# Arieys/MonteCarloPathTracing

Hardware: AMD Instinct MI355X
Metric: Mrays/s on cornell-box 1280x720 SPP=256 (closest-hit queries actually traced / wall time incl. gather) (higher is better)
Workload: dtype f64

## Files before the change

montecarlopathtracing_amd/csrc/kernels.hip:

```cpp
#include <hip/hip_runtime.h>

#include "accel_build.hpp"
#include "dev_common.hpp"
#include "kernels.hpp"
#include "shade_common.hpp"
#include "shade_path.hpp"
#include "trace_persistent.hpp"
#include "trace_pool.hpp"

namespace mcpt {

template <bool LEAF>
__global__ void __launch_bounds__(256) k_trace_closest_reference(DScene S, const double* __restrict__ rays, long long n,
                                                       int32_t* __restrict__ face, double* __restrict__ t_out,
                                                       double* __restrict__ p_out, double* __restrict__ pn_out, DCounters* ctr)
{
    const long long gid = (long long)blockIdx.x * blockDim.x + threadIdx.x;
    LaneStats ls;
    if (gid < n) {
        Ray r;
        r.o = ld3(rays + gid * 6); r.d = ld3(rays + gid * 6 + 3);
        Hit h; Work w = {0, 0};
        const bool ok = trace_closest(S, r, h, w);
        ls.nodes = w.nodes; ls.tris = w.tris; ls.primary = 1;
        V3 pn = mk(0, 0, 0);
        if (ok && !LEAF) pn = hit_normal(S, h);
        if (face) face[gid] = ok ? (LEAF ? h.leaf : S.tris[h.leaf].face) : -1;
        if (t_out) t_out[gid] = ok ? h.t : 0.0;
        if (p_out) { p_out[gid * 3] = h.p.x; p_out[gid * 3 + 1] = h.p.y; p_out[gid * 3 + 2] = h.p.z; }
        if (pn_out) { pn_out[gid * 3] = pn.x; pn_out[gid * 3 + 1] = pn.y; pn_out[gid * 3 + 2] = pn.z; }
    }
    flush_stats(ctr, ls);
}

struct ArrayRaySource {
    static constexpr bool kWantsPoint = true;
    const double* rays; long long n;
    int32_t* leaf_out; double* t_out; double* p_out;
    __device__ __forceinline__ long long total() const { return n; }
    __device__ __forceinline__ bool fetch(long long q, Ray& r) const
    {
        r.o = ld3(rays + q * 6); r.d = ld3(rays + q * 6 + 3);
#ifdef MCPT_DBG_INVALID
        return ((((unsigned int)q * 2654435761u) >> 7) & 3u) != 0u;
#else
        return true;
#endif
    }
    __device__ __forceinline__ void store(long long q, bool ok, const Hit& h) const
    {
        leaf_out[q] = ok ? h.leaf : -1;
        t_out[q] = ok ? h.t : 0.0;
        p_out[q * 3] = h.p.x; p_out[q * 3 + 1] = h.p.y; p_out[q * 3 + 2] = h.p.z;
    }
};

struct PrimaryRaySource {
    static constexpr bool kWantsPoint = true;
    const double* dirs; const int32_t* pixels; int n_pixels; double eye[3]; PrimaryHit* hits;
    __device__ __forceinline__ long long total() const { return n_pixels; }
    __device__ __forceinline__ bool fetch(long long q, Ray& r) const
    {
        const int pix = pixels ? pixels[q] : (int)q;
        r.o = ld3(eye); r.d = ld3(dirs + (size_t)pix * 3);
        return true;
    }
    __device__ __forceinline__ void store(long long q, bool ok, const Hit& h) const
    {
        PrimaryHit ph;
        ph.leaf = ok ? h.leaf : -1; ph.surf = 0; ph.t = h.t; ph.p[0] = h.p.x; ph.p[1] = h.p.y; ph.p[2] = h.p.z;
        hits[q] = ph;
    }
};

template <class Src, int STACK, int WAVES>
__global__ void __launch_bounds__(256, WAVES) k_trace_persistent(DScene S, Src src, TraceQueue* queue, long long* slow_list, unsigned int slow_cap,
                                                                long long chunk, DCounters* ctr)
{
    __shared__ int lds_stack[STACK * 256];
    __shared__ double lds_rays[4 * MCPT_RAYBUF_BYTES / 8];
    LaneStats ls;
    Work w = {0, 0};
    trace_persistent(S, src, queue, slow_list, slow_cap, chunk, lds_stack + threadIdx.x, 256, lds_rays + (threadIdx.x >> 6) * (MCPT_RAYBUF_BYTES / 8), w, S.fast.stack_cap < STACK ? S.fast.stack_cap : STACK);
    ls.nodes = w.nodes; ls.tris = w.tris;
    { const unsigned long long tw = wave_sum(w.pre_wrong); if ((threadIdx.x & 63) == 0 && tw && ctr) atomicAdd(&ctr->pre_wrong, tw); }
    flush_stats(ctr, ls);
}

template <class Src, int NW, int KT, int SCAP>
__global__ void __launch_bounds__(NW * 64, 1) k_trace_pool(DScene S, Src src, TraceQueue* queue, long long* slow_list, unsigned int slow_cap,
                                                          long long chunk, DCounters* ctr)
{
    __shared__ PoolLds<NW, KT, SCAP> L;
    LaneStats ls;
    Work w = {0, 0};
    trace_pool<Src, NW, KT, SCAP>(S, src, queue, slow_list, slow_cap, chunk, L, w, reinterpret_cast<int*>(slow_list + slow_cap));
    ls.nodes = w.nodes; ls.tris = w.tris;
    { const unsigned long long tw = wave_sum(w.pre_wrong); if ((threadIdx.x & 63) == 0 && tw && ctr) atomicAdd(&ctr->pre_wrong, tw); }
    flush_stats(ctr, ls);
}

template <class Src>
__global__ void __launch_bounds__(256) k_trace_slow(DScene S, Src src, const TraceQueue* queue, const long long* slow_list, unsigned int slow_cap,
                                                    DCounters* ctr)
{
    __shared__ int lds_stack[MCPT_FAST_STACK * 256];
    LaneStats ls;
    Work w = {0, 0};
    trace_slow_list(S, src, queue, slow_list, slow_cap, w, lds_stack + threadIdx.x);
    ls.nodes = w.nodes; ls.tris = w.tris;
    flush_stats(ctr, ls);
}

__global__ void k_finish_hits(DScene S, long long n, int32_t* __restrict__ face, const double* __restrict__ p, double* __restrict__ pn_out, DCounters* ctr)
{
    const long long gid = (long long)blockIdx.x * blockDim.x + threadIdx.x;
    LaneStats ls;
    if (gid < n) {
        ls.primary = 1;
        const int leaf = face[gid];
        V3 pn = mk(0, 0, 0);
        if (leaf >= 0) {
            Hit h; h.leaf = leaf; h.t = 0; h.p = ld3(p + gid * 3);
            pn = hit_normal(S, h);
            face[gid] = S.tris[leaf].face;
        }
        if (pn_out) { pn_out[gid * 3] = pn.x; pn_out[gid * 3 + 1] = pn.y; pn_out[gid * 3 + 2] = pn.z; }
    }
    flush_stats(ctr, ls);
}

__global__ void k_primary_dirs(DCamera cam, double* __restrict__ dirs)
{
    const int row = blockIdx.x * blockDim.x + threadIdx.x;
    if (row >= cam.height) return;
    const V3 eye = ld3(cam.eye), pdx = ld3(cam.pdx);
    V3 pos = ld3(cam.start_point) - ld3(cam.pdy) * (double)row;
    double* out = dirs + (size_t)row * cam.width * 3;
    for (int j = 0; j < cam.width; j++) {
        const V3 d = normalized(pos - eye);
        out[j * 3] = d.x; out[j * 3 + 1] = d.y; out[j * 3 + 2] = d.z;
// ... 484 lines not shown
```

montecarlopathtracing_amd/csrc/trace_pool.hpp:

```cpp
#pragma once
#include "env.hpp"
#include "trace_persistent.hpp"
#include "vertex.hpp"

namespace mcpt {

struct NoPaths { static constexpr bool kPaths = false; };

#ifndef MCPT_POOL_WAVES
#define MCPT_POOL_WAVES 16
#endif
#ifndef MCPT_POOL_KT
#define MCPT_POOL_KT 20
#endif
#ifndef MCPT_POOL_STACK
#define MCPT_POOL_STACK 8
#endif
#define MCPT_POOL_SPILL (MCPT_FAST_STACK - MCPT_POOL_STACK)
#ifndef MCPT_POOL_CLAIMS
#define MCPT_POOL_CLAIMS 2
#endif
#define MCPT_POOL_CLAIM_ORDER __ATOMIC_ACQUIRE
#define MCPT_POOL_FILE_ORDER __ATOMIC_RELEASE

struct alignas(16) PoolOxy { double ox, oy; };
struct alignas(16) PoolOzDx { double oz, dx; };
struct alignas(16) PoolDyz { double dy, dz; };
struct alignas(16) PoolRcp { float rx, ry, rz, limit; };
typedef double pool_d2 __attribute__((ext_vector_type(2)));
template <class T>
__device__ __forceinline__ T pool_ld16(const T* p)
{
    static_assert(sizeof(T) == 16, "16-byte group");
    const pool_d2 v = *reinterpret_cast<const pool_d2*>(p);
    T r;
    __builtin_memcpy(&r, &v, 16);
    return r;
}

template <int NW, int KT, int SCAP>
struct PoolLds {
    PoolOxy oxy[KT * 64];
    PoolOzDx ozdx[KT * 64];
    PoolDyz dyz[KT * 64];
    PoolRcp rcp[KT * 64];
    double best_t[KT * 64];
    unsigned int q[KT * 64];
    int cur[KT * 64];
    int best_leaf[KT * 64];
    int spf[KT * 64];
    int stack[SCAP * KT * 64];
    unsigned int cls[5 * 64];
    unsigned int busy[64];
    int tbl[NW * 64];
    unsigned int stat[8];
    unsigned int live;
    unsigned int dry;
};

__device__ __forceinline__ int uni(int v) { return __builtin_amdgcn_readfirstlane(v); }
__device__ __forceinline__ long long uni(long long v)
{
    const int lo = __builtin_amdgcn_readfirstlane((int)(unsigned int)(unsigned long long)v);
    const int hi = __builtin_amdgcn_readfirstlane((int)(unsigned int)((unsigned long long)v >> 32));
    return (long long)(((unsigned long long)(unsigned int)hi << 32) | (unsigned int)lo);
}

template <class Src, int NW, int KT, int SCAP, class PP = NoPaths>
__device__ __forceinline__ void trace_pool(const DScene& S, const Src& src, TraceQueue* queue, long long* __restrict__ slow_list,
                                           unsigned int slow_cap, long long chunk, PoolLds<NW, KT, SCAP>& L, Work& w,
                                           int* __restrict__ spill ,
                                           const PP& pp = PP())
{
    static_assert(KT <= 32, "one 32-bit set per class");
    static_assert(SCAP >= 6, "the pushes of a ray's first two steps land in LDS");
    enum { C_INNER = 0, C_LEAF = 1, C_EXACT = 2, C_FIN = 3, C_SHADE = 4, C_DEAD = 5 };
    enum { F_FOUND = 256, F_AMBIG = 512, F_RAY = 1024, F_OWNFAIL = 2048  };
    const DFast& F = S.fast;
    const CwNode* __restrict__ nodes = F.cw;
    const DTri* __restrict__ tris = F.tris;
    const DTriPre* __restrict__ pre = F.pre;
    const TicketSchedule ts = make_ticket_schedule(src.total(), chunk);
    const int lane = threadIdx.x & 63, wave = uni((int)(threadIdx.x >> 6));
    const int stack_max = spill ? SCAP + MCPT_POOL_SPILL : SCAP;
    const int stack_cap = F.stack_cap < stack_max ? F.stack_cap : stack_max;
    int* __restrict__ my_spill = spill ? spill + (size_t)blockIdx.x * MCPT_POOL_SPILL * (KT * 64) : nullptr;
    auto st_put = [&](int e, int k, int v) __attribute__((always_inline)) {
        if (e < SCAP) L.stack[(e * KT + k) * 64 + lane] = v;
        else my_spill[((e - SCAP) * KT + k) * 64 + lane] = v;
    };
    auto st_get = [&](int e, int k) __attribute__((always_inline)) -> int {
        return e < SCAP ? L.stack[(e * KT + k) * 64 + lane] : my_spill[((e - SCAP) * KT + k) * 64 + lane];
    };

    for (int k = wave; k < KT; k += NW) { L.spf[k * 64 + lane] = 0; if constexpr (PP::kPaths) L.q[k * 64 + lane] = 0u; }
    int R = 1, NP = KT;
    if constexpr (PP::kPaths) { R = pp.nl + 1; NP = KT / R; }
    if (wave == 0) {
        L.cls[C_INNER * 64 + lane] = 0u; L.cls[C_LEAF * 64 + lane] = 0u; L.cls[C_EXACT * 64 + lane] = 0u;
        L.cls[C_FIN * 64 + lane] = PP::kPaths ? 0u : (unsigned int)((1ull << KT) - 1ull);
        L.cls[C_SHADE * 64 + lane] = PP::kPaths ? (unsigned int)((1ull << NP) - 1ull) : 0u;
        L.busy[lane] = 0u;
    }
    if (threadIdx.x == 0) { L.live = (PP::kPaths ? NP : KT) * 64; L.dry = 0; }
    if (threadIdx.x < 8) L.stat[threadIdx.x] = 0u;
    __syncthreads();

    unsigned int c_nodes = 0, c_rays = 0, c_exact = 0;
#ifdef MCPT_POOL_DEBUG
    unsigned long long d_used = 0, d_okc = 0, d_steps = 0, d_kill = 0, d_tickets = 0;
    unsigned long long d_cs[5] = {0, 0, 0, 0, 0}, d_cl[5] = {0, 0, 0, 0, 0}, d_sleep = 0, d_miss = 0, d_want[5] = {0, 0, 0, 0, 0};
    unsigned long long d_cyc[6] = {0, 0, 0, 0, 0, 0};
    unsigned long long d_t = __builtin_amdgcn_s_memtime();
    const unsigned long long d_t0 = d_t;
#endif
    long long next = 0, range_end = 0;
    bool queue_empty = false;
    int rot = wave % KT;
    const int rot_stride = (int)((0x13110d0bu >> (8 * ((wave >> 1) & 3))) & 255u) % KT | 1;
    const float s3f = __double2float_ru(3.0 * F.absmax), absmax_f = __double2float_ru(F.absmax);
    auto pad_of = [&](float of, float rf_) __attribute__((always_inline)) { return (0x1p-20f * 1.00001f) * ((fabsf(of) + s3f) * fabsf(rf_)); };
    auto margin_of = [&](const float of[3], const PoolRcp& a4) __attribute__((always_inline)) {
        const float rmax = fmaxf(fmaxf(fabsf(a4.rx), fabsf(a4.ry)), fabsf(a4.rz));
        const float scale = fmaxf(fmaxf(absmax_f, fabsf(of[0])), fmaxf(fabsf(of[1]), fabsf(of[2])));
        return rmax <= 0.99e6f ? (1.0000001e-9f * 1.00001f) * (scale * rmax) : __builtin_inff();
    };
    auto pop_next = [&](int idx, int k, int spf) __attribute__((always_inline)) -> int {
        int sp = spf & 255;
        if (sp == 0) return C_FIN;
        sp--;
        int nxt;
        if (!__ballot(sp >= SCAP)) { nxt = L.stack[(sp * KT + k) * 64 + lane]; __asm__ volatile("" : "+v"(nxt)); }
        else nxt = st_get(sp, k);
        const bool node = nxt >= 0;
        const int ref = -1 - nxt;
        const int first = node ? nxt : ref >> 4, cnt = (ref & 7) + 1;
        L.cur[idx] = first;
        L.spf[idx] = (spf & 0xff00) | sp | (node ? 0 : cnt << 16);
        return node ? C_INNER : C_LEAF;
    };

    for (;;) {
        const unsigned int m_inner = __hip_atomic_load(&L.cls[C_INNER * 64 + lane], __ATOMIC_RELAXED, __HIP_MEMORY_SCOPE_WORKGROUP);
        const unsigned int m_leaf = __hip_atomic_load(&L.cls[C_LEAF * 64 + lane], __ATOMIC_RELAXED, __HIP_MEMORY_SCOPE_WORKGROUP);
        const unsigned int m_exact = __hip_atomic_load(&L.cls[C_EXACT * 64 + lane], __ATOMIC_RELAXED, __HIP_MEMORY_SCOPE_WORKGROUP);
        const unsigned int m_fin = __hip_atomic_load(&L.cls[C_FIN * 64 + lane], __ATOMIC_RELAXED, __HIP_MEMORY_SCOPE_WORKGROUP);
        const int n_inner = __popcll(__ballot(m_inner != 0u));
        const int n_leaf = __popcll(__ballot(m_leaf != 0u));
        const int n_exact = __popcll(__ballot(m_exact != 0u));
        const bool fin_ok = PP::kPaths || !queue_empty || uni((int)__hip_atomic_load(&L.dry, __ATOMIC_RELAXED, __HIP_MEMORY_SCOPE_WORKGROUP)) == NW;
        const int n_fin = fin_ok ? __popcll(__ballot(m_fin != 0u)) : 0;
        unsigned int m_shade = 0u;
        int n_shade = 0;
        if constexpr (PP::kPaths) {
            m_shade = __hip_atomic_load(&L.cls[C_SHADE * 64 + lane], __ATOMIC_RELAXED, __HIP_MEMORY_SCOPE_WORKGROUP);
            n_shade = __popcll(__ballot(m_shade != 0u));
        }
        if (!(n_inner | n_leaf | n_exact | n_fin | n_shade)) {
            if (uni((int)__hip_atomic_load(&L.live, __ATOMIC_RELAXED, __HIP_MEMORY_SCOPE_WORKGROUP)) == 0) break;
            __builtin_amdgcn_s_sleep(4);
#ifdef MCPT_POOL_DEBUG
            d_sleep++;
#endif
            continue;
        }
        int c = C_FIN, best_score = n_fin;
        if (n_exact > best_score) { c = C_EXACT; best_score = n_exact; }
        if (n_leaf > best_score) { c = C_LEAF; best_score = n_leaf; }
        if (n_inner > best_score) { c = C_INNER; best_score = n_inner; }
        if (PP::kPaths && n_shade >= best_score && n_shade) { c = C_SHADE; best_score = n_shade; }
        c = uni(c);

        bool have = false;
        int k = 0;
        unsigned int cm = c == C_INNER ? m_inner : (c == C_LEAF ? m_leaf : (c == C_EXACT ? m_exact : (c == C_FIN ? m_fin : m_shade)));
        unsigned int* const cword = &L.cls[c * 64 + lane];
        const unsigned int below = 0xffffffffu >> (31 - rot), above = 0xffffffffu << rot;
#pragma unroll
        for (int attempt = 0; attempt < MCPT_POOL_CLAIMS; attempt++) {
            const bool want = !have && cm != 0u;
            if (attempt && !__ballot(want)) break;
            if (want) {
                int kk;
                if (wave & 1) { const unsigned int lo = cm & below; kk = 31 - __clz((int)(lo ? lo : cm)); }
                else { const unsigned int hi = cm & above; kk = __ffs((int)(hi ? hi : cm)) - 1; }
                const unsigned int bit = 1u << kk;
                const unsigned int old = __hip_atomic_fetch_and(cword, ~bit, MCPT_POOL_CLAIM_ORDER, __HIP_MEMORY_SCOPE_WORKGROUP);
                have = (old & bit) != 0u;
                k = kk;
                cm = old & ~bit;
            }
        }
        { rot += rot_stride; if (rot >= KT) rot -= KT; }
        const unsigned long long hv = __ballot(have);
#ifdef MCPT_POOL_DEBUG
        if (!hv) d_miss++;
#endif
        if (!hv) continue;
        const int n_have = __popcll(hv);
// ... 277 lines not shown
                            else p = ldc(a.out.p, cap, j);
                            for (int l = 0; l < nl; l++) {
                                const int expect = a.out.expect[(long long)l * cap + j];
                                ri[(size_t)(RI_EXPECT + l) * plane] = expect;
                                if (expect != -2) {
                                    const V3 cc = ldc(a.out.c + (long long)l * 3 * cap, cap, j), d = ldc(a.rays.d + (long long)l * 3 * cap, cap, j);
                                    stp(RD_C + 3 * l, cc); emit(s0 + l, p + d * 0.01, d);
                                }
                            }
                            const int bt = a.out.btype[j];
                            ri[RI_BT * plane] = bt;
                            if (bt >= 0) {
                                const V3 bd = ldc(a.out.bdir, cap, j);
                                if (!folded) stp(RD_W, ldc(a.out.w, cap, j));
                                emit(s0 + nl, (bt & MCPT_BT_NO_OFFSET) ? p : p + bd * 0.01, bd);
                            }
                            ri[RI_ID * plane] = id; ri[RI_DEPTH * plane] = (int)depth;
                            stp(RD_T, T); stp(RD_L, Lr);
                            mode = P_ADOPTED;
                        } else dead = true;
                    }
                }
                if (have) {
                    L.q[s0 * 64 + lane] = (unsigned int)mode;
                    const unsigned int nb = nb_inner | nb_fin;
                    if (nb) __hip_atomic_fetch_or(&L.busy[lane], nb, __ATOMIC_RELAXED, __HIP_MEMORY_SCOPE_WORKGROUP);
                    if (nb_inner) __hip_atomic_fetch_or(&L.cls[C_INNER * 64 + lane], nb_inner, MCPT_POOL_FILE_ORDER, __HIP_MEMORY_SCOPE_WORKGROUP);
                    if (nb_fin) __hip_atomic_fetch_or(&L.cls[C_FIN * 64 + lane], nb_fin, MCPT_POOL_FILE_ORDER, __HIP_MEMORY_SCOPE_WORKGROUP);
                    nc = (mode != P_FREE && !nb) ? C_SHADE : C_DEAD;
                    w.rays += (unsigned int)__popc(nb);
                }
                const int n_dead = __popcll(__ballot(have && dead));
                if (n_dead && lane == 0) __hip_atomic_fetch_sub(&L.live, (unsigned int)n_dead, __ATOMIC_RELAXED, __HIP_MEMORY_SCOPE_WORKGROUP);
                const unsigned int t_sh = (unsigned int)wave_sum((unsigned long long)n_shadow), t_sk = (unsigned int)wave_sum((unsigned long long)n_skipped),
                                   t_bo = (unsigned int)wave_sum((unsigned long long)n_bounce);
                if (lane == 0) {
                    if (n_shades) atomicAdd(&L.stat[0], (unsigned int)n_shades);
                    if (t_sh) atomicAdd(&L.stat[1], t_sh);
                    if (t_bo) atomicAdd(&L.stat[2], t_bo);
                    if (t_sk) atomicAdd(&L.stat[3], t_sk);
                    if (deepest) atomicMax(&L.stat[4], deepest);
                }
            }
        } else {
            if (have) {
                const int spf = L.spf[idx];
                if (spf & F_RAY) {
                    const PoolOxy a0 = pool_ld16(&L.oxy[idx]); const PoolOzDx a1 = pool_ld16(&L.ozdx[idx]); const PoolDyz a2 = pool_ld16(&L.dyz[idx]);
                    const long long slot = (long long)L.q[idx];
                    Ray r; r.o = mk(a0.ox, a0.oy, a1.oz); r.d = mk(a1.dx, a2.dy, a2.dz);
                    const bool found = (spf & F_FOUND) != 0;
                    bool ambiguous = (spf & F_AMBIG) != 0;
                    Hit h; h.leaf = -1; h.t = 0; h.p = mk(0, 0, 0);
                    if (found) {
                        const DTri* tr = tris + L.best_leaf[idx];
                        if (spf & F_OWNFAIL) ambiguous = true;
                        h.leaf = tr->leaf;
                        h.mat = tr->material;
                        h.p = hit_point(tr, r);
                        h.t = (h.p.x - r.o.x) / r.d.x;
                    }
                    if (ambiguous) defer_ray(queue, slow_list, slow_cap, slot, true);
                    else src.store(slot, found, h);
                }
            }
            bool got = false;
            bool all_dry = queue_empty;
            if (!queue_empty && next >= range_end) {
                unsigned long long tk = 0;
                if (lane == 0) tk = atomicAdd(&queue->head, 1ull);
                const bool in_range = ticket_range(ts, uni((long long)tk), next, range_end);
#ifdef MCPT_POOL_DEBUG
                d_tickets++;
#endif
                if (!in_range) {
                    queue_empty = true;
                    unsigned int before = 0;
                    if (lane == 0) before = __hip_atomic_fetch_add(&L.dry, 1u, __ATOMIC_RELAXED, __HIP_MEMORY_SCOPE_WORKGROUP);
                    all_dry = uni((int)before) + 1 == NW;
                }
            }
            if (!queue_empty) {
                const long long left = range_end - next;
                const int avail = left < 64 ? (int)left : 64;
                Ray nr; nr.o = mk(0, 0, 0); nr.d = mk(1, 1, 1);
                const bool valid = lane < avail && src.fetch(next + lane, nr);
                const bool ok = valid && fast_path_ok(F, nr);
                const unsigned long long V = __ballot(ok);
                const int n_ok = __popcll(V);
                const int rank_ok = (int)__builtin_amdgcn_mbcnt_hi((unsigned int)(V >> 32), __builtin_amdgcn_mbcnt_lo((unsigned int)V, 0u));
                int used = avail;
                if (n_ok > n_have) used = __ffsll((long long)__ballot(ok && rank_ok == n_have - 1));
                used = uni(used);
                if (valid && !ok && lane < used) defer_ray(queue, slow_list, slow_cap, next + lane, false);
                if (ok && rank_ok < n_have) L.tbl[wave * 64 + rank_ok] = lane;
                const int rank_need = (int)__builtin_amdgcn_mbcnt_hi((unsigned int)(hv >> 32), __builtin_amdgcn_mbcnt_lo((unsigned int)hv, 0u));
                got = have && rank_need < n_ok;
                __asm__ volatile("" ::: "memory");
                const int from = got ? L.tbl[wave * 64 + rank_need] : lane;
                CwNodeWords root = (CwNodeWords)nodes;
                __asm__ volatile("" : "+s"(root));
                Ray r;
                r.o.x = __shfl(nr.o.x, from, 64); r.o.y = __shfl(nr.o.y, from, 64); r.o.z = __shfl(nr.o.z, from, 64);
                r.d.x = __shfl(nr.d.x, from, 64); r.d.y = __shfl(nr.d.y, from, 64); r.d.z = __shfl(nr.d.z, from, 64);
                bool second = false;
                if (got) {
                    const V3 rcp = mk(fast_rcp(r.d.x), fast_rcp(r.d.y), fast_rcp(r.d.z));
                    PoolOxy b0; b0.ox = r.o.x; b0.oy = r.o.y;
                    PoolOzDx b1; b1.oz = r.o.z; b1.dx = r.d.x;
                    PoolDyz b2; b2.dy = r.d.y; b2.dz = r.d.z;
                    PoolRcp b4; b4.rx = (float)rcp.x; b4.ry = (float)rcp.y; b4.rz = (float)rcp.z; b4.limit = __builtin_inff();
                    L.oxy[idx] = b0; L.ozdx[idx] = b1; L.dyz[idx] = b2; L.rcp[idx] = b4;
                    L.best_t[idx] = 0;
                    L.best_leaf[idx] = -1;
                    L.q[idx] = (unsigned int)(next + from);
                    {
                        RayF rf;
                        rf.o[0] = (float)b0.ox; rf.o[1] = (float)b0.oy; rf.o[2] = (float)b1.oz;
                        rf.r[0] = b4.rx; rf.r[1] = b4.ry; rf.r[2] = b4.rz;
                        rf.pad[0] = pad_of(rf.o[0], b4.rx); rf.pad[1] = pad_of(rf.o[1], b4.ry); rf.pad[2] = pad_of(rf.o[2], b4.rz);
                        int* const col = &L.stack[k * 64 + lane];
                        int sp = 0;
                        auto push_hits = [&](const CwHits& h) __attribute__((always_inline)) -> int {
                            const int n_hit = (h.ref[0] != MCPT_FAST_EMPTY) + (h.ref[1] != MCPT_FAST_EMPTY) + (h.ref[2] != MCPT_FAST_EMPTY) + (h.ref[3] != MCPT_FAST_EMPTY);
                            if (n_hit >= 4) col[sp * (KT * 64)] = h.ref[3];
                            if (n_hit >= 3) col[(sp + n_hit - 3) * (KT * 64)] = h.ref[2];
                            if (n_hit >= 2) col[(sp + n_hit - 2) * (KT * 64)] = h.ref[1];
                            sp += n_hit > 1 ? n_hit - 1 : 0;
                            int nx = h.ref[0];
                            if (nx == MCPT_FAST_EMPTY && sp > 0) { sp--; nx = col[sp * (KT * 64)]; }
                            return nx;
                        };
                        int nxt = push_hits(cw_step_uniform(root, rf));
                        second = nxt >= 0 && !(sp > stack_cap - 3);
                        if (second) nxt = push_hits(cw_step(nodes + nxt, rf, __builtin_inff()));
                        const bool node = nxt >= 0, none = nxt == MCPT_FAST_EMPTY;
                        const int ref = -1 - nxt;
                        L.cur[idx] = none ? 0 : (node ? nxt : ref >> 4);
                        L.spf[idx] = F_RAY | sp | ((!node && !none) ? ((ref & 7) + 1) << 16 : 0);
                        nc = node ? C_INNER : (none ? C_FIN : C_LEAF);
                    }
                }
                next += used;
#ifdef MCPT_POOL_DEBUG
                d_used += used; d_okc += __popcll(__ballot(ok && lane < used)); d_steps++;
#endif
                const unsigned int n_got = (unsigned int)__popcll(__ballot(got));
                c_rays += n_got;
                c_nodes += n_got + (unsigned int)__popcll(__ballot(got && second));
            }
            if (have && !got) {
                if (queue_empty && all_dry) nc = C_DEAD;
                else { L.spf[idx] = 0; nc = C_FIN; }
            }
            const int n_dead = __popcll(__ballot(have && nc == C_DEAD));
#ifdef MCPT_POOL_DEBUG
            d_kill += n_dead;
#endif
            if (n_dead && lane == 0) __hip_atomic_fetch_sub(&L.live, (unsigned int)n_dead, __ATOMIC_RELAXED, __HIP_MEMORY_SCOPE_WORKGROUP);
        }
        __asm__ volatile("" ::: "memory");
#ifdef MCPT_POOL_DEBUG
        { const unsigned long long tn = __builtin_amdgcn_s_memtime(); d_cyc[c] += tn - d_t; d_t = tn; }
#endif
        if (have && nc != C_DEAD)
            __hip_atomic_fetch_or(&L.cls[nc * 64 + lane], 1u << k, MCPT_POOL_FILE_ORDER, __HIP_MEMORY_SCOPE_WORKGROUP);
    }
    if (lane == 0) { w.nodes += c_nodes; w.rays += c_rays; w.exact += c_exact; }
#ifdef MCPT_POOL_DEBUG
    if constexpr (PP::kPaths) {
        if (lane == 0 && pp.a.ctr) {
            PoolAccount& o = pp.a.ctr->dbg.account;
            for (int i = 0; i < 5; i++) { atomicAdd(&o.steps[i], d_cs[i]); atomicAdd(&o.lanes[i], d_cl[i]); atomicAdd(&o.cycles[i], d_cyc[i]); }
            atomicAdd(&o.sleeps, d_sleep); atomicAdd(&o.missed, d_miss); atomicAdd(&o.overhead, d_cyc[5]);
            atomicAdd(&o.life, __builtin_amdgcn_s_memtime() - d_t0); atomicAdd(&o.waves, 1ull);
        }
    } else
    if (lane == 0 && w.dbg) {
        {
            PoolAccount& o = w.dbg->account;
            for (int i = 0; i < 4; i++) { atomicAdd(&o.steps[i], d_cs[i]); atomicAdd(&o.lanes[i], d_cl[i]); atomicAdd(&o.cycles[i], d_cyc[i]); }
            atomicAdd(&o.sleeps, d_sleep); atomicAdd(&o.missed, d_miss); atomicAdd(&o.overhead, d_cyc[5]);
            atomicAdd(&o.life, __builtin_amdgcn_s_memtime() - d_t0); atomicAdd(&o.waves, 1ull);
        }
        PoolDebug& g = w.dbg->pool;
        atomicAdd(&g.used, d_used); atomicAdd(&g.ok, d_okc); atomicAdd(&g.refills, d_steps); atomicAdd(&g.retired, d_kill); atomicAdd(&g.tickets, d_tickets);
        atomicAdd(&g.started, (unsigned long long)c_rays);
        for (int i = 0; i < 4; i++) { atomicAdd(&g.class_steps[i], d_cs[i]); atomicAdd(&g.class_lanes[i], d_cl[i]); atomicAdd(&g.class_want[i], d_want[i]); }
        atomicAdd(&g.sleeps, d_sleep); atomicAdd(&g.missed, d_miss);
        if (threadIdx.x == 0 && blockIdx.x == 0) { atomicAdd(&g.slots, (unsigned long long)ts.total); atomicAdd(&g.launches, 1ull); }
    }
#endif
}

}
```

montecarlopathtracing_amd/csrc/wavefront.hip:

```cpp
#include <hip/hip_runtime.h>

#include <cstdio>
#include <cstdlib>
#include <cstring>

#include "accel_build.hpp"
#include "dev_common.hpp"
#include "shade_common.hpp"
#include "trace_persistent.hpp"
#include "trace_pool.hpp"
#include "vertex.hpp"
#include "wavefront.hpp"
#include "wf_ray_source.hpp"

namespace mcpt {

size_t wf_bytes_per_path(int nl)
{
    const size_t state = 4 + (6 + 3 * nl + (nl == 1 ? 3 : 6)) * 8 + nl * 4 + 4 + nl * 4 + 4 + 3 * 8;
    const size_t rays = nl * 3 * 8;
    return 2 * state + rays;
}

bool wf_carve(void* base, size_t bytes, long long cap, int nl, WfState& A, WfState& B, WfRays& R)
// ... 113 lines not shown
    Work w = {0, 0};
    trace_slow_list(S, src, queue, slow_list, slow_cap, w, lds_stack + threadIdx.x);
    ls.nodes = w.nodes; ls.tris = w.tris;
    flush_stats(a.ctr, ls);
}

__global__ void __launch_bounds__(256) k_wf_trace_reference(DScene S, WfArgs a)
{
    const long long n_paths = a.counts->n_next;
    WfRaySource src; src.a = a; src.n_paths = n_paths;
    const long long total = src.total();
    LaneStats ls;
    Work w = {0, 0};
    for (long long q = (long long)blockIdx.x * 256 + threadIdx.x; q < total; q += (long long)gridDim.x * 256) {
        Ray r;
        if (!src.fetch(q, r)) continue;
        Hit h;
        const bool ok = trace_closest(S, r, h, w);
        src.store(q, ok, h);
    }
    ls.nodes = w.nodes; ls.tris = w.tris;
    flush_stats(a.ctr, ls);
}

static unsigned grid_for(long long n, int block, unsigned cap_blocks)
{
    long long b = (n + block - 1) / block;
    if (b < 1) b = 1;
    return (unsigned)(b > cap_blocks ? cap_blocks : b);
}

bool pool_engine_available()
{
    static const int ok = [] {
        int per_cu = 0;
        const hipError_t e = hipOccupancyMaxActiveBlocksPerMultiprocessor(
            &per_cu, reinterpret_cast<const void*>(k_wf_trace_pool<MCPT_POOL_WAVES, MCPT_POOL_KT, MCPT_POOL_STACK>), MCPT_POOL_WAVES * 64, 0);
        if (e != hipSuccess) (void)hipGetLastError();
        return (e == hipSuccess && per_cu >= 1 && pool_engine_available_closest()) ? 1 : 0;
    }();
    return ok != 0;
}

size_t pool_spill_bytes(int cus)
{
    return size_t(cus > 0 ? cus : 256) * size_t(MCPT_POOL_SPILL) * size_t(MCPT_POOL_KT * 64) * sizeof(int);
}

int persistent_grid(const void* kernel, int cus)
{
    int per_cu = 0;
    if (hipOccupancyMaxActiveBlocksPerMultiprocessor(&per_cu, kernel, 256, 0) != hipSuccess || per_cu <= 0) per_cu = 4;
    return cus * per_cu;
}

void init_launch_cfg(LaunchCfg& cfg, unsigned forced_logic_grid, long long trace_block_rays, int min_chunk, int max_chunk)
{
    int dev = 0;
    hipDeviceProp_t prop;
    cfg.cus = 0;
    if (hipGetDevice(&dev) == hipSuccess && hipGetDeviceProperties(&prop, dev) == hipSuccess) cfg.cus = prop.multiProcessorCount;
    if (cfg.cus <= 0) cfg.cus = 256;
    init_launch_cfg_logic(cfg, forced_logic_grid);
    cfg.trace_grid = persistent_grid(reinterpret_cast<const void*>(k_wf_trace<MCPT_FAST_STACK, 3>), cfg.cus);
    cfg.trace_grid_short = persistent_grid(reinterpret_cast<const void*>(k_wf_trace<kFastShortStack, 4>), cfg.cus);
    cfg.trace_block_rays = trace_block_rays >= 256 ? trace_block_rays : 2048;
    cfg.min_chunk = min_chunk >= 64 ? min_chunk / 64 * 64 : 256;
    cfg.max_chunk = max_chunk >= 64 ? max_chunk / 64 * 64 : 2048;
    if (cfg.max_chunk < cfg.min_chunk) cfg.max_chunk = cfg.min_chunk;
    cfg.trace_pool = 0;
    init_launch_cfg_closest(cfg);
}

long long persistent_chunk(long long total, int grid_blocks)
{
    const long long waves = (long long)grid_blocks * 4;
    long long c = total / (waves * 4);
    c = (c / 64) * 64;
    if (c < 64) c = 64;
    if (c > 2048) c = 2048;
    return c;
}

void launch_wf_trace(const DScene& S, const WfArgs& a, long long n_upper, bool fast, TraceQueue* queue, long long* slow_list,
                     unsigned int slow_cap, hipStream_t st, const LaunchCfg& cfg)
{
    if (n_upper <= 0) return;
    const long long total = n_upper * (a.nl + 1);
    if (!fast) {
        hipLaunchKernelGGL(k_wf_trace_reference, dim3(grid_for(total, 256, 1u << 20)), dim3(256), 0, st, S, a);
        return;
    }
    const bool shallow = S.fast.stack_limit <= kFastShortStack;
    const int resident = shallow ? cfg.trace_grid_short : cfg.trace_grid;
    const long long blocks_needed = (total + cfg.trace_block_rays - 1) / cfg.trace_block_rays;
    const int g = (int)(blocks_needed < resident ? blocks_needed : resident);
    if (a.queue != queue) (void)hipMemsetAsync(queue, 0, sizeof(TraceQueue), st);
    if (cfg.trace_pool && total < (1ll << 32)) {
        const long long per_block = cfg.trace_block_rays * (MCPT_POOL_WAVES / 4);
        const long long nb = (total + per_block - 1) / per_block;
        const int gp = (int)(nb < cfg.cus ? nb : cfg.cus);
        hipLaunchKernelGGL((k_wf_trace_pool<MCPT_POOL_WAVES, MCPT_POOL_KT, MCPT_POOL_STACK>), dim3(gp), dim3(MCPT_POOL_WAVES * 64), 0, st, S, a, queue, slow_list, slow_cap, cfg.min_chunk, cfg.max_chunk);
    } else if (shallow) hipLaunchKernelGGL((k_wf_trace<kFastShortStack, 4>), dim3(g), dim3(256), 0, st, S, a, queue, slow_list, slow_cap, cfg.min_chunk, cfg.max_chunk);
    else hipLaunchKernelGGL((k_wf_trace<MCPT_FAST_STACK, 3>), dim3(g), dim3(256), 0, st, S, a, queue, slow_list, slow_cap, cfg.min_chunk, cfg.max_chunk);
    hipLaunchKernelGGL(k_wf_trace_slow, dim3(g < 512 ? g : 512), dim3(256), 0, st, S, a, queue, slow_list, slow_cap);
}

}
```

montecarlopathtracing_amd/csrc/wavefront.hpp:

```cpp
#pragma once
#include <hip/hip_runtime_api.h>

#include "device_scene.hpp"
#include "kernels.hpp"

namespace mcpt {

struct WfState {
    int32_t* id;
    double* T;
    double* L;
    double* c;
    int32_t* expect;
    double* w;
    double* bdir;
    int32_t* btype;
    int32_t* hit_mat;
    int32_t* hit_leaf;
    double* p;
};

struct WfRays {
    double* d;
};

struct alignas(16) PrimarySurface {
    double p[3], dir[3];
    double pn[3], kd[3];
    int32_t leaf, material, pixel, slot;
    int32_t alive_index, pad[3];
};

#define MCPT_HIT_EMITTER 0x40000000
#define MCPT_HIT_LEAF_MASK 0x3fffffff

struct TraceQueue {
    unsigned long long head;
    unsigned int slow_count;
    unsigned int redo_all;
    unsigned int pad[12];
};

struct WfCounts {
    unsigned int n_next;
    unsigned int finish_claimed;
    unsigned int pad1;
    unsigned int shaded_pixels;
    unsigned int pad[12];
};
static_assert(sizeof(WfCounts) == 64 && offsetof(WfCounts, finish_claimed) == 4 && offsetof(WfCounts, shaded_pixels) == 12, "one 64-byte segment; the words the kernels share");
#define MCPT_WF_COUNT_SLOTS 72

struct WfArgs {
    WfState in, out;
    WfRays rays;
    long long cap;
    int nl, spp, depth;
    unsigned long long seed;
    const int32_t* pixels;
    const int32_t* hit_slots;
    const PrimarySurface* surf;
    const unsigned int* alive_base;
    PrimaryHit* hits;
    const double* dirs;
    int first_slot;
    double* rad;
    WfCounts* counts;
    const WfCounts* counts_in;
    unsigned int count_mul;
    DCounters* ctr;
    const DTri* tris;
    const DMaterial* materials;
    unsigned int finish_below;
    TraceQueue* queue;
    int sample_base;
    uint8_t* cam_hit;
};

size_t wf_bytes_per_path(int nl);
bool wf_carve(void* base, size_t bytes, long long cap, int nl, WfState& a, WfState& b, WfRays& r);

void launch_wf_logic(const DScene& S, const WfArgs& a, long long n_upper, bool first, hipStream_t st, const LaunchCfg& cfg);
void launch_wf_trace(const DScene& S, const WfArgs& a, long long n_upper, bool fast, TraceQueue* queue, long long* slow_list,
                     unsigned int slow_cap, hipStream_t st, const LaunchCfg& cfg);
void launch_wf_finish(const DScene& S, const WfArgs& a, long long n_upper, hipStream_t st, const LaunchCfg& cfg, char* path_area, long long* slow_list,
                      unsigned int slow_cap);
size_t finish_pool_bytes(int cus, int nl);
int persistent_grid(const void* kernel, int cus);
void init_launch_cfg_logic(LaunchCfg& cfg, unsigned forced_grid);
long long persistent_chunk(long long total, int grid_blocks);

void launch_primary_surface(const DScene& S, const WfArgs& a, PrimarySurface* surf, unsigned int* alive_count, unsigned int* alive_total, int n_slots_upper,
                            hipStream_t st);
void launch_hit_slots(const PrimaryHit* hits, int first_slot, int n_slots, int32_t* hit_slots, unsigned int* count, hipStream_t st);
void launch_zero_rad(double* rad, long long n_doubles, hipStream_t st);
void launch_camera_pass(const DLens& lens, const WfArgs& a, long long n_samples, hipStream_t st);
void launch_query_pass(const DQuery& q, const WfArgs& a, long long n_samples, hipStream_t st);

}
```

montecarlopathtracing_amd/csrc/wf_ray_source.hpp:

```cpp
#pragma once
#include "dev_common.hpp"
#include "vertex.hpp"
#include "wavefront.hpp"

namespace mcpt {

struct WfRaySource {
    static constexpr bool kWantsPoint = false;
    WfArgs a;
    long long n_paths;
    __device__ __forceinline__ long long total() const { return n_paths * (a.nl + 1); }
    __device__ __forceinline__ void split(long long q, int& l, long long& j) const
    {
        l = 0; j = q;
        while (j >= n_paths) { j -= n_paths; l++; }
    }
    __device__ __forceinline__ V3 vertex(long long j) const
    {
        if (a.depth == 0 && a.hits) {
            const PrimaryHit* ph = a.hits + (a.first_slot + a.out.id[j] / a.spp);
            return mk(ph->p[0], ph->p[1], ph->p[2]);
        }
        return ldc(a.out.p, a.cap, j);
    }
    __device__ __forceinline__ bool fetch(long long q, Ray& r) const
    {
        int l; long long j;
        split(q, l, j);
        const bool bounce = l == a.nl;
        const int flag = bounce ? a.out.btype[j] : a.out.expect[(long long)l * a.cap + j];
        const V3 p = vertex(j);
        r.d = ldc(bounce ? a.out.bdir : a.rays.d + (long long)l * 3 * a.cap, a.cap, j);
        r.o = (bounce && (flag & MCPT_BT_NO_OFFSET)) ? p : p + r.d * 0.01;
        return bounce ? flag >= 0 : flag != -2;
    }
    __device__ __forceinline__ void store(long long q, bool ok, const Hit& h) const
    {
        int l; long long j;
        split(q, l, j);
        if (l == a.nl) {
            int v = -1;
            if (ok) { const int mat = h.mat >= 0 ? h.mat : a.tris[h.leaf].material; v = h.leaf | (a.materials[mat].light >= 0 ? MCPT_HIT_EMITTER : 0); }
            a.out.hit_leaf[j] = v;
        } else {
            a.out.hit_mat[(long long)l * a.cap + j] = ok ? (h.mat >= 0 ? h.mat : a.tris[h.leaf].material) : -1;
        }
    }
};

typedef const WfArgs __attribute__((address_space(4)))* WfArgsKernarg;
template <class T> __device__ __forceinline__ const T __attribute__((address_space(1)))* wf_glob(const T* p)
{
    return (const T __attribute__((address_space(1)))*)p;
}
template <class T> __device__ __forceinline__ T __attribute__((address_space(1)))* wf_glob_mut(T* p)
{
    return (T __attribute__((address_space(1)))*)p;
}
#ifndef MCPT_TRACE_NT
#define MCPT_TRACE_NT 0
#endif
#if MCPT_TRACE_NT
template <class P> __device__ __forceinline__ auto wf_sld(P p) { return __builtin_nontemporal_load(p); }
template <class P, class T> __device__ __forceinline__ void wf_sst(P p, T v) { __builtin_nontemporal_store(v, p); }
#else
template <class P> __device__ __forceinline__ auto wf_sld(P p) { return *p; }
template <class P, class T> __device__ __forceinline__ void wf_sst(P p, T v) { *p = v; }
#endif
struct WfRaySourceK {
    static constexpr bool kWantsPoint = false;
    WfArgsKernarg ap;
    long long n_paths;
    int nl;
    __device__ __forceinline__ WfArgsKernarg args() const { WfArgsKernarg p = ap; __asm__ volatile("" : "+s"(p)); return p; }
    __device__ __forceinline__ long long total() const { return n_paths * (nl + 1); }
    __device__ __forceinline__ void split(long long q, int& l, long long& j) const
    {
        l = 0; j = q;
        while (j >= n_paths) { j -= n_paths; l++; }
    }
    __device__ __forceinline__ bool fetch(long long q, Ray& r) const
    {
        int l; long long j;
        split(q, l, j);
        const WfArgsKernarg A = args();
        const long long cap = A->cap;
        const bool bounce = l == nl;
        const int flag = bounce ? wf_sld(wf_glob(A->out.btype) + j) : wf_sld(wf_glob(A->out.expect) + ((long long)l * cap + j));
        V3 p;
        if (A->depth == 0 && A->hits) {
            const auto* ph = wf_glob(A->hits) + (A->first_slot + wf_glob(A->out.id)[j] / A->spp);
            p = mk(ph->p[0], ph->p[1], ph->p[2]);
        } else {
            const auto* g = wf_glob(A->out.p);
            p = mk(wf_sld(g + j), wf_sld(g + cap + j), wf_sld(g + 2 * cap + j));
        }
        const auto* d = wf_glob(bounce ? A->out.bdir : A->rays.d + (long long)l * 3 * cap);
        r.d = mk(wf_sld(d + j), wf_sld(d + cap + j), wf_sld(d + 2 * cap + j));
        r.o = (bounce && (flag & MCPT_BT_NO_OFFSET)) ? p : p + r.d * 0.01;
        return bounce ? flag >= 0 : flag != -2;
    }
    __device__ __forceinline__ void store(long long q, bool ok, const Hit& h) const
    {
        int l; long long j;
        split(q, l, j);
        const WfArgsKernarg A = args();
        if (l == nl) {
            int v = -1;
            if (ok) { const int mat = h.mat >= 0 ? h.mat : wf_glob(A->tris)[h.leaf].material; v = h.leaf | (wf_glob(A->materials)[mat].light >= 0 ? MCPT_HIT_EMITTER : 0); }
            wf_sst(wf_glob_mut(A->out.hit_leaf) + j, v);
        }
        else wf_sst(wf_glob_mut(A->out.hit_mat) + ((long long)l * A->cap + j), ok ? (h.mat >= 0 ? h.mat : wf_glob(A->tris)[h.leaf].material) : -1);
    }
};

}
```

Before: 5660.

## Add adaptive 128-wide sparse refill window for wavefront trace pool

For sparse wavefront ray sources, the persistent trace pool can now scan a 128-entry window of flags and compact only valid rays into idle lanes, fetching full ray data only for lanes that take one. This avoids loading ray origins and directions for slots that carry no ray. The kernel switches adaptively between window mode and the old 64-lane fetch based on observed density. It also replaces the per-ray integer divide by spp with a host-computed magic multiply. The cost is extra flag loads, ballots and LDS traffic, plus more code and register pressure in the refill path.

```diff
diff --git a/montecarlopathtracing_amd/csrc/kernels.hip b/montecarlopathtracing_amd/csrc/kernels.hip
--- a/montecarlopathtracing_amd/csrc/kernels.hip
+++ b/montecarlopathtracing_amd/csrc/kernels.hip
@@ -35,6 +35,7 @@
 
 struct ArrayRaySource {
     static constexpr bool kWantsPoint = true;
+    static constexpr bool kSparse = false;
     const double* rays; long long n;
     int32_t* leaf_out; double* t_out; double* p_out;
     __device__ __forceinline__ long long total() const { return n; }
@@ -57,6 +58,7 @@
 
 struct PrimaryRaySource {
     static constexpr bool kWantsPoint = true;
+    static constexpr bool kSparse = false;
     const double* dirs; const int32_t* pixels; int n_pixels; double eye[3]; PrimaryHit* hits;
     __device__ __forceinline__ long long total() const { return n_pixels; }
     __device__ __forceinline__ bool fetch(long long q, Ray& r) const
diff --git a/montecarlopathtracing_amd/csrc/refill_window.hpp b/montecarlopathtracing_amd/csrc/refill_window.hpp
--- /dev/null
+++ b/montecarlopathtracing_amd/csrc/refill_window.hpp
@@ -0,0 +1,71 @@
+#pragma once
+
+namespace mcpt {
+
+#ifdef __HIPCC__
+#define MCPT_RW_FN __host__ __device__ __forceinline__
+#else
+#define MCPT_RW_FN inline
+#endif
+
+enum { kRefillWindow = 128 };
+
+MCPT_RW_FN int refill_n_valid(unsigned long long V0, unsigned long long V1)
+{
+    return __builtin_popcountll(V0) + __builtin_popcountll(V1);
+}
+
+MCPT_RW_FN int refill_rank(unsigned long long V0, int half, int below_in_half)
+{
+    return (half ? __builtin_popcountll(V0) : 0) + below_in_half;
+}
+MCPT_RW_FN int refill_below(unsigned long long V, int lane)
+{
+    return __builtin_popcountll(V & ((1ull << lane) - 1ull));
+}
+
+MCPT_RW_FN bool refill_taken(int rank, int n_have) { return rank < n_have; }
+MCPT_RW_FN bool refill_last(int rank, int n_have) { return rank == n_have - 1; }
+
+MCPT_RW_FN int refill_used(unsigned long long last0, unsigned long long last1, int n_valid, int n_have, int W)
+{
+    if (n_valid <= n_have) return W;
+    return last0 ? __builtin_ctzll(last0) + 1 : 64 + __builtin_ctzll(last1) + 1;
+}
+
+struct DivMagic { unsigned int mul; int shift; };
+MCPT_RW_FN DivMagic div_magic(unsigned int d)
+{
+    int l = 0;
+    while ((1ull << l) < d) l++;
+    DivMagic r;
+    r.mul = (unsigned int)((1ull << (31 + l)) / d + 1ull);
+    r.shift = 31 + l;
+    return r;
+}
+MCPT_RW_FN unsigned int div_by_magic(unsigned int n, unsigned int mul, int shift)
+{
+    return (unsigned int)(((unsigned long long)n * mul) >> shift);
+}
+
+#ifndef __HIP_DEVICE_COMPILE__
+inline int refill_window(unsigned long long V0, unsigned long long V1, int n_have, int W, unsigned char off[64], int* n_take)
+{
+    const int n_valid = refill_n_valid(V0, V1);
+    unsigned long long last[2] = {0ull, 0ull};
+    const unsigned long long V[2] = {V0, V1};
+    for (int half = 0; half < 2; half++)
+        for (int lane = 0; lane < 64; lane++) {
+            if (!((V[half] >> lane) & 1ull)) continue;
+            const int rank = refill_rank(V0, half, refill_below(V[half], lane));
+            if (refill_taken(rank, n_have)) off[rank] = (unsigned char)(half * 64 + lane);
+            if (refill_last(rank, n_have)) last[half] |= 1ull << lane;
+        }
+    *n_take = n_valid < n_have ? n_valid : n_have;
+    return refill_used(last[0], last[1], n_valid, n_have, W);
+}
+#endif
+
+#undef MCPT_RW_FN
+
+}
diff --git a/montecarlopathtracing_amd/csrc/trace_pool.hpp b/montecarlopathtracing_amd/csrc/trace_pool.hpp
--- a/montecarlopathtracing_amd/csrc/trace_pool.hpp
+++ b/montecarlopathtracing_amd/csrc/trace_pool.hpp
@@ -1,5 +1,6 @@
 #pragma once
 #include "env.hpp"
+#include "refill_window.hpp"
 #include "trace_persistent.hpp"
 #include "vertex.hpp"
 
@@ -115,6 +116,7 @@
     const unsigned long long d_t0 = d_t;
 #endif
     long long next = 0, range_end = 0;
+    [[maybe_unused]] bool window_next = true;
     bool queue_empty = false;
     int rot = wave % KT;
     const int rot_stride = (int)((0x13110d0bu >> (8 * ((wave >> 1) & 3))) & 255u) % KT | 1;
@@ -558,27 +560,75 @@
             }
             if (!queue_empty) {
                 const long long left = range_end - next;
-                const int avail = left < 64 ? (int)left : 64;
-                Ray nr; nr.o = mk(0, 0, 0); nr.d = mk(1, 1, 1);
-                const bool valid = lane < avail && src.fetch(next + lane, nr);
-                const bool ok = valid && fast_path_ok(F, nr);
-                const unsigned long long V = __ballot(ok);
-                const int n_ok = __popcll(V);
-                const int rank_ok = (int)__builtin_amdgcn_mbcnt_hi((unsigned int)(V >> 32), __builtin_amdgcn_mbcnt_lo((unsigned int)V, 0u));
-                int used = avail;
-                if (n_ok > n_have) used = __ffsll((long long)__ballot(ok && rank_ok == n_have - 1));
-                used = uni(used);
-                if (valid && !ok && lane < used) defer_ray(queue, slow_list, slow_cap, next + lane, false);
-                if (ok && rank_ok < n_have) L.tbl[wave * 64 + rank_ok] = lane;
                 const int rank_need = (int)__builtin_amdgcn_mbcnt_hi((unsigned int)(hv >> 32), __builtin_amdgcn_mbcnt_lo((unsigned int)hv, 0u));
-                got = have && rank_need < n_ok;
-                __asm__ volatile("" ::: "memory");
-                const int from = got ? L.tbl[wave * 64 + rank_need] : lane;
                 CwNodeWords root = (CwNodeWords)nodes;
                 __asm__ volatile("" : "+s"(root));
-                Ray r;
-                r.o.x = __shfl(nr.o.x, from, 64); r.o.y = __shfl(nr.o.y, from, 64); r.o.z = __shfl(nr.o.z, from, 64);
-                r.d.x = __shfl(nr.d.x, from, 64); r.d.y = __shfl(nr.d.y, from, 64); r.d.z = __shfl(nr.d.z, from, 64);
+                Ray r; r.o = mk(0, 0, 0); r.d = mk(1, 1, 1);
+                int from = lane;
+                int used;
+#ifdef MCPT_POOL_DEBUG
+                int n_okc;
+#endif
+                bool use_window = false;
+                if constexpr (Src::kSparse) use_window = window_next;
+                if (use_window) {
+                  if constexpr (Src::kSparse) {
+                    const int W = left < (long long)kRefillWindow ? (int)left : (int)kRefillWindow;
+                    int win_l; long long win_j;
+                    src.split(next, win_l, win_j);
+                    win_l = uni(win_l); win_j = uni(win_j);
+                    int flag0 = 0, flag1 = 0;
+                    bool fb0 = false, fb1 = false;
+                    { int l; long long j;
+                      if (lane < W) { src.split_from(win_l, win_j, lane, l, j); flag0 = src.flag(l, j, fb0); }
+                      if (lane + 64 < W) { src.split_from(win_l, win_j, 64 + lane, l, j); flag1 = src.flag(l, j, fb1); } }
+                    const bool v0 = lane < W && Src::flag_has_ray(flag0, fb0);
+                    const bool v1 = lane + 64 < W && Src::flag_has_ray(flag1, fb1);
+                    const unsigned long long V0 = __ballot(v0), V1 = __ballot(v1);
+                    const int n_valid = refill_n_valid(V0, V1);
+                    const int rank0 = refill_rank(V0, 0, (int)__builtin_amdgcn_mbcnt_hi((unsigned int)(V0 >> 32), __builtin_amdgcn_mbcnt_lo((unsigned int)V0, 0u)));
+                    const int rank1 = refill_rank(V0, 1, (int)__builtin_amdgcn_mbcnt_hi((unsigned int)(V1 >> 32), __builtin_amdgcn_mbcnt_lo((unsigned int)V1, 0u)));
+                    if (v0 && refill_taken(rank0, n_have)) L.tbl[wave * 64 + rank0] = lane;
+                    if (v1 && refill_taken(rank1, n_have)) L.tbl[wave * 64 + rank1] = 64 + lane;
+                    used = uni(refill_used(__ballot(v0 && refill_last(rank0, n_have)), __ballot(v1 && refill_last(rank1, n_have)), n_valid, n_have, W));
+                    const bool take = have && rank_need < n_valid;
+                    __asm__ volatile("" ::: "memory");
+                    if (take) {
+                        from = L.tbl[wave * 64 + rank_need];
+                        int l; long long j;
+                        src.split_from(win_l, win_j, from, l, j);
+                        src.fetch(l, j, r);
+                        got = fast_path_ok(F, r);
+                        if (!got) defer_ray(queue, slow_list, slow_cap, next + from, false);
+                    }
+                    window_next = (n_valid < n_have ? n_valid : n_have) * 8 < used * 7;
+#ifdef MCPT_POOL_DEBUG
+                    n_okc = __popcll(__ballot(got));
+#endif
+                  }
+                } else {
+                    const int avail = left < 64 ? (int)left : 64;
+                    Ray nr; nr.o = mk(0, 0, 0); nr.d = mk(1, 1, 1);
+                    const bool valid = lane < avail && src.fetch(next + lane, nr);
+                    const bool ok = valid && fast_path_ok(F, nr);
+                    const unsigned long long V = __ballot(ok);
+                    const int n_ok = __popcll(V);
+                    const int rank_ok = (int)__builtin_amdgcn_mbcnt_hi((unsigned int)(V >> 32), __builtin_amdgcn_mbcnt_lo((unsigned int)V, 0u));
+                    used = avail;
+                    if (n_ok > n_have) used = __ffsll((long long)__ballot(ok && rank_ok == n_have - 1));
+                    used = uni(used);
+                    if (valid && !ok && lane < used) defer_ray(queue, slow_list, slow_cap, next + lane, false);
+                    if (ok && rank_ok < n_have) L.tbl[wave * 64 + rank_ok] = lane;
+                    got = have && rank_need < n_ok;
+                    __asm__ volatile("" ::: "memory");
+                    from = got ? L.tbl[wave * 64 + rank_need] : lane;
+                    r.o.x = __shfl(nr.o.x, from, 64); r.o.y = __shfl(nr.o.y, from, 64); r.o.z = __shfl(nr.o.z, from, 64);
+                    r.d.x = __shfl(nr.d.x, from, 64); r.d.y = __shfl(nr.d.y, from, 64); r.d.z = __shfl(nr.d.z, from, 64);
+                    if constexpr (Src::kSparse) window_next = __popcll(__ballot(valid && lane < used)) * 8 < used * 7;
+#ifdef MCPT_POOL_DEBUG
+                    n_okc = __popcll(__ballot(ok && lane < used));
+#endif
+                }
                 bool second = false;
                 if (got) {
                     const V3 rcp = mk(fast_rcp(r.d.x), fast_rcp(r.d.y), fast_rcp(r.d.z));
@@ -619,7 +669,7 @@
                 }
                 next += used;
 #ifdef MCPT_POOL_DEBUG
-                d_used += used; d_okc += __popcll(__ballot(ok && lane < used)); d_steps++;
+                d_used += used; d_okc += n_okc; d_steps++;
 #endif
                 const unsigned int n_got = (unsigned int)__popcll(__ballot(got));
                 c_rays += n_got;
diff --git a/montecarlopathtracing_amd/csrc/wavefront.hip b/montecarlopathtracing_amd/csrc/wavefront.hip
--- a/montecarlopathtracing_amd/csrc/wavefront.hip
+++ b/montecarlopathtracing_amd/csrc/wavefront.hip
@@ -219,10 +219,12 @@
     return c;
 }
 
-void launch_wf_trace(const DScene& S, const WfArgs& a, long long n_upper, bool fast, TraceQueue* queue, long long* slow_list,
+void launch_wf_trace(const DScene& S, const WfArgs& args, long long n_upper, bool fast, TraceQueue* queue, long long* slow_list,
                      unsigned int slow_cap, hipStream_t st, const LaunchCfg& cfg)
 {
     if (n_upper <= 0) return;
+    WfArgs a = args;
+    { const DivMagic dm = div_magic((unsigned int)(a.spp > 0 ? a.spp : 1)); a.spp_mul = dm.mul; a.spp_shift = dm.shift; }
     const long long total = n_upper * (a.nl + 1);
     if (!fast) {
         hipLaunchKernelGGL(k_wf_trace_reference, dim3(grid_for(total, 256, 1u << 20)), dim3(256), 0, st, S, a);
diff --git a/montecarlopathtracing_amd/csrc/wavefront.hpp b/montecarlopathtracing_amd/csrc/wavefront.hpp
--- a/montecarlopathtracing_amd/csrc/wavefront.hpp
+++ b/montecarlopathtracing_amd/csrc/wavefront.hpp
@@ -75,6 +75,8 @@
     TraceQueue* queue;
     int sample_base;
     uint8_t* cam_hit;
+    unsigned int spp_mul;
+    int spp_shift;
 };
 
 size_t wf_bytes_per_path(int nl);
diff --git a/montecarlopathtracing_amd/csrc/wf_ray_source.hpp b/montecarlopathtracing_amd/csrc/wf_ray_source.hpp
--- a/montecarlopathtracing_amd/csrc/wf_ray_source.hpp
+++ b/montecarlopathtracing_amd/csrc/wf_ray_source.hpp
@@ -1,5 +1,6 @@
 #pragma once
 #include "dev_common.hpp"
+#include "refill_window.hpp"
 #include "vertex.hpp"
 #include "wavefront.hpp"
 
@@ -7,6 +8,7 @@
 
 struct WfRaySource {
     static constexpr bool kWantsPoint = false;
+    static constexpr bool kSparse = true;
     WfArgs a;
     long long n_paths;
     __device__ __forceinline__ long long total() const { return n_paths * (a.nl + 1); }
@@ -23,10 +25,33 @@
         }
         return ldc(a.out.p, a.cap, j);
     }
+    __device__ __forceinline__ void split_from(int l0, long long j0, int off, int& l, long long& j) const
+    {
+        l = l0; j = j0 + off;
+        while (j >= n_paths) { j -= n_paths; l++; }
+    }
+    __device__ __forceinline__ int flag(int l, long long j, bool& bounce) const
+    {
+        bounce = l == a.nl;
+        return bounce ? a.out.btype[j] : a.out.expect[(long long)l * a.cap + j];
+    }
+    static __device__ __forceinline__ bool flag_has_ray(int flag, bool bounce) { return bounce ? flag >= 0 : flag != -2; }
+    __device__ __forceinline__ bool has_ray(long long q) const
+    {
+        int l; long long j;
+        split(q, l, j);
+        bool bounce;
+        const int f = flag(l, j, bounce);
+        return flag_has_ray(f, bounce);
+    }
     __device__ __forceinline__ bool fetch(long long q, Ray& r) const
     {
         int l; long long j;
         split(q, l, j);
+        return fetch(l, j, r);
+    }
+    __device__ __forceinline__ bool fetch(int l, long long j, Ray& r) const
+    {
         const bool bounce = l == a.nl;
         const int flag = bounce ? a.out.btype[j] : a.out.expect[(long long)l * a.cap + j];
         const V3 p = vertex(j);
@@ -69,6 +94,7 @@
 #endif
 struct WfRaySourceK {
     static constexpr bool kWantsPoint = false;
+    static constexpr bool kSparse = true;
     WfArgsKernarg ap;
     long long n_paths;
     int nl;
@@ -79,17 +105,41 @@
         l = 0; j = q;
         while (j >= n_paths) { j -= n_paths; l++; }
     }
+    __device__ __forceinline__ void split_from(int l0, long long j0, int off, int& l, long long& j) const
+    {
+        l = l0; j = j0 + off;
+        while (j >= n_paths) { j -= n_paths; l++; }
+    }
+    __device__ __forceinline__ int flag(int l, long long j, bool& bounce) const
+    {
+        const WfArgsKernarg A = args();
+        bounce = l == nl;
+        return bounce ? wf_sld(wf_glob(A->out.btype) + j) : wf_sld(wf_glob(A->out.expect) + ((long long)l * A->cap + j));
+    }
+    static __device__ __forceinline__ bool flag_has_ray(int flag, bool bounce) { return bounce ? flag >= 0 : flag != -2; }
+    __device__ __forceinline__ bool has_ray(long long q) const
+    {
+        int l; long long j;
+        split(q, l, j);
+        bool bounce;
+        const int f = flag(l, j, bounce);
+        return flag_has_ray(f, bounce);
+    }
     __device__ __forceinline__ bool fetch(long long q, Ray& r) const
     {
         int l; long long j;
         split(q, l, j);
+        return fetch(l, j, r);
+    }
+    __device__ __forceinline__ bool fetch(int l, long long j, Ray& r) const
+    {
         const WfArgsKernarg A = args();
         const long long cap = A->cap;
         const bool bounce = l == nl;
         const int flag = bounce ? wf_sld(wf_glob(A->out.btype) + j) : wf_sld(wf_glob(A->out.expect) + ((long long)l * cap + j));
         V3 p;
         if (A->depth == 0 && A->hits) {
-            const auto* ph = wf_glob(A->hits) + (A->first_slot + wf_glob(A->out.id)[j] / A->spp);
+            const auto* ph = wf_glob(A->hits) + (A->first_slot + (int)div_by_magic((unsigned int)wf_glob(A->out.id)[j], A->spp_mul, A->spp_shift));
             p = mk(ph->p[0], ph->p[1], ph->p[2]);
         } else {
             const auto* g = wf_glob(A->out.p);
```

Result: faster. 5824 (median of 6 runs) (+2.9%).
